# yflyzhang/RankPO

Hardware: AMD Instinct MI355X
Metric: query-passage pairs/sec (higher is better)
Workload: dtype bf16

## Files before the change

include/rankpo_hip.h:

```cpp
#ifndef RANKPO_HIP_H
#define RANKPO_HIP_H

#include <stddef.h>
#include <stdint.h>

#ifdef __cplusplus
extern "C" {
#endif

typedef void* rpo_stream_t;

typedef enum {
    RPO_OK = 0,
    RPO_ERR_INVALID_ARG = -1,
    RPO_ERR_UNSUPPORTED = -2,
    RPO_ERR_WORKSPACE = -3,
    RPO_ERR_LAUNCH = -4
} rpo_status;

typedef enum { RPO_DT_F32 = 0, RPO_DT_BF16 = 1, RPO_DT_F16 = 2 } rpo_dtype;
typedef enum { RPO_POOL_LAST = 0, RPO_POOL_CLS = 1 } rpo_pool_mode;
typedef enum { RPO_TARGET_INBATCH = 0, RPO_TARGET_FIRST = 1 } rpo_target_mode;
typedef enum { RPO_LOSS_SIGMOID = 0, RPO_LOSS_HINGE = 1 } rpo_loss_type;

// ... 70 lines not shown

typedef enum {
    RPO_LS_SCALE = 0,
    RPO_LS_MULT = 1,
    RPO_LS_NORM = 2,
    RPO_LS_SKIP = 3,
    RPO_LS_GOOD_STEPS = 4,
    RPO_LS_CUR_HYSTERESIS = 5,
    RPO_LS_APPLIED_STEPS = 6,
    RPO_LS_SKIPPED_STEPS = 7,
    RPO_LS_FLOOR_HITS = 8,
    RPO_LS_WORDS = 16
} rpo_ls_word;
int rpo_loss_scale_update(const float* sumsq, void* ls_state, float pre_scale, float max_grad_norm, int dynamic, int window,
                          int hysteresis, int consecutive_hysteresis, float min_scale, rpo_stream_t stream);
int rpo_adamw_step_scaled(void* param, float* master, const void* grad, float* exp_avg, float* exp_avg_sq, int64_t n,
                          int dtype, float lr, float beta1, float beta2, float eps, float weight_decay, const void* ls_state,
                          rpo_stream_t stream);

int rpo_swiglu_fwd(const void* g, const void* u, void* out, int64_t rows, int64_t cols, int64_t ld_gu, int64_t ld_out,
                   int dtype, rpo_stream_t stream);
int rpo_swiglu_bwd(const void* g, const void* u, const void* dout, void* dg, void* du, void* prod_out, int64_t rows,
                   int64_t cols, int64_t ld_gu, int64_t ld_dout, int64_t ld_dgu, int64_t ld_prod, int dtype,
                   rpo_stream_t stream);
int rpo_swiglu_bwd_t(const void* g, const void* u, const void* dout, void* dg, void* du, void* prod_t_out, void* dgu_t_out,
                     int64_t rows, int64_t cols, int64_t ld_gu, int64_t ld_dout, int64_t ld_dgu, int64_t ld_t, int dtype,
                     rpo_stream_t stream);
int rpo_rope(const void* x_in, void* x_out, int64_t row_stride, const float* cos_tab, const float* sin_tab,
             int64_t rows, int64_t heads, int64_t head_dim, int64_t period, int dtype, int backward,
             rpo_stream_t stream);

int rpo_transpose(const void* in, void* out, int64_t rows, int64_t cols, int64_t ld_in, int64_t ld_out, int dtype,
                  rpo_stream_t stream);

int rpo_add_rmsnorm_waves(int64_t rows);
int rpo_add_rmsnorm_fwd(const void* x, const void* delta, const void* weight, float eps, void* x_out, void* y_out,
                        float* rstd_out, int64_t rows, int64_t d, int dtype, rpo_stream_t stream);
int rpo_add_rmsnorm_bwd(const void* dy, const void* x_new, const void* weight, const float* rstd, const void* dres,
                        void* dx_out, float* dw_partial, int64_t rows, int64_t d, int dtype, rpo_stream_t stream);

int rpo_flash_attn_fwd(const void* q, const void* k, const void* v, int64_t q_stride, int64_t k_stride,
                       int64_t v_stride, const int* cu_seqlens, const int* tiles, int64_t ntiles, int64_t tile_cols,
                       int64_t total_tokens,
                       int64_t num_heads, int64_t num_kv_heads, int64_t head_dim, float scale, void* out,
                       int64_t out_stride, float* lse, int64_t lse_max_len, const float* rope_cos, const float* rope_sin,
                       int64_t rope_period, int64_t q_block, rpo_stream_t stream);

int rpo_flash_attn_bwd(const void* q, const void* k, const void* v, const void* out, const void* dout, int64_t q_stride,
                       int64_t k_stride, int64_t v_stride, int64_t out_stride, int64_t dout_stride,
                       const int* cu_seqlens, const int* q_tiles, int64_t n_q_tiles, int64_t q_tile_cols, const int* k_tiles,
                       int64_t n_k_tiles, int64_t key_block, int64_t sweep_down, int64_t total_tokens, int64_t num_heads,
                       int64_t num_kv_heads, int64_t head_dim, float scale, const float* lse, float* delta, void* dq, void* dk, void* dv,
                       int64_t dq_stride, int64_t dk_stride, int64_t dv_stride, const float* rope_cos, const float* rope_sin,
                       int64_t rope_period, int64_t q_block, rpo_stream_t stream);

int rpo_lastq_attn_fwd(const void* q, int64_t q_stride, const void* k, const void* v, int64_t k_stride, int64_t v_stride,
                       const int* cu_seqlens, int64_t num_seqs, int64_t num_heads, int64_t num_kv_heads, int64_t head_dim,
                       float scale, void* out, int64_t out_stride, float* lse, rpo_stream_t stream);
int rpo_lastq_attn_bwd(const void* q, int64_t q_stride, const void* k, const void* v, int64_t k_stride, int64_t v_stride,
                       const int* cu_seqlens, int64_t num_seqs, int64_t num_heads, int64_t num_kv_heads, int64_t head_dim,
                       float scale, const void* out, int64_t out_stride, const void* dout, int64_t dout_stride, const float* lse,
                       void* dq, int64_t dq_stride, void* dk, void* dv, int64_t dk_stride, int64_t dv_stride, rpo_stream_t stream);

int rpo_bidir_attn_fwd(const void* q, const void* k, const void* v, int64_t q_stride, int64_t k_stride, int64_t v_stride,
                       const int* cu_seqlens_q, const int* cu_seqlens_k, const int* tiles, int64_t ntiles, int64_t tile_cols,
                       int64_t q_block, int64_t total_q, int64_t num_heads, int64_t num_kv_heads, int64_t head_dim, int dtype,
// ... 94 lines not shown
```

rankpo_amd/_lib.py:

```python
from __future__ import annotations

import ctypes as C
import os

_HERE = os.path.dirname(os.path.abspath(__file__))
LIB_PATH = os.path.join(_HERE, "csrc", "librankpo_hip.so")

RPO_OK = 0
RPO_DT_F32, RPO_DT_BF16, RPO_DT_F16 = 0, 1, 2
RPO_POOL_LAST, RPO_POOL_CLS = 0, 1
(RPO_LS_SCALE, RPO_LS_MULT, RPO_LS_NORM, RPO_LS_SKIP, RPO_LS_GOOD_STEPS, RPO_LS_CUR_HYSTERESIS, RPO_LS_APPLIED_STEPS,
 RPO_LS_SKIPPED_STEPS, RPO_LS_FLOOR_HITS) = range(9)
RPO_LS_WORDS = 16
RPO_TARGET_INBATCH, RPO_TARGET_FIRST = 0, 1
RPO_LOSS_SIGMOID, RPO_LOSS_HINGE = 0, 1
RPO_BUILD_ONEWAVE64 = 1
RPO_NUM_METRICS = 9
METRIC_KEYS = (
    "rankpo_loss", "sft_loss", "rewards/chosen", "rewards/rejected", "rewards/accuracies",
    "rewards/margins", "scores/chosen", "scores/rejected", "scores/margins",
)


class RankPOParams(C.Structure):
# ... 14 lines not shown
    "rpo_version": (C.c_int, []),
    "rpo_build_flags": (C.c_int, []),
    "rpo_status_string": (C.c_char_p, [C.c_int]),
    "rpo_last_hip_error": (C.c_char_p, []),
    "rpo_pool_normalize_fwd": (C.c_int, [_vp, _i64, _i64, _vp, _i64, _i64, _i64, _i32, _i32, _i32, _f32, _vp, _vp, _vp, _vp]),
    "rpo_pool_normalize_bwd": (C.c_int, [_vp, _vp, _vp, _vp, _i64, _i64, _i64, _i32, _i32, _f32, _vp, _vp, _vp]),
    "rpo_infonce_workspace_bytes": (_sz, [_i64, _i64, _i64, _i32]),
    "rpo_infonce_debug_poison_tickets": (C.c_int, [C.c_uint64, _vp]),
    "rpo_infonce_fwd": (C.c_int, [_vp, _vp, _i64, _i64, _i64, _i32, _f32, _i32, _vp, _vp, _vp, _vp, _sz, _vp]),
    "rpo_infonce_bwd": (C.c_int, [_vp, _vp, _vp, _vp, _vp, _i64, _i64, _i64, _i32, _f32, _i32, _i64, _i64, _i64, _i64,
                                  _vp, _vp, _vp, _sz, _vp]),
    "rpo_infonce_ds": (C.c_int, [_vp, _vp, _vp, _i64, _i64, _i32, _f32, _i64, _i64, _i64, _i64, _vp, _vp, _vp]),
    "rpo_sim_gemm_nt": (C.c_int, [_vp, _i64, _i64, _vp, _i64, _i64, _i64, _vp, _i64, _vp]),
    "rpo_rankpo_fwd": (C.c_int, [_vp, _vp, _vp, _vp, _i64, _i64, _i32, C.POINTER(RankPOParams), _vp, _vp, _vp, _vp, _vp, _vp]),
    "rpo_rankpo_bwd": (C.c_int, [_vp, _vp, _vp, _vp, _i64, _i64, _i32, _vp, _vp, _vp]),
    "rpo_adamw_step": (C.c_int, [_vp, _vp, _vp, _vp, _vp, _i64, _i32, _f32, _f32, _f32, _f32, _f32, _f32, _f32, _vp, _vp]),
    "rpo_sumsq_partial": (C.c_int, [_vp, _i64, _i32, _vp, _i32, _vp]),
    "rpo_loss_scale_update": (C.c_int, [_vp, _vp, _f32, _f32, _i32, _i32, _i32, _i32, _f32, _vp]),
    "rpo_adamw_step_scaled": (C.c_int, [_vp, _vp, _vp, _vp, _vp, _i64, _i32, _f32, _f32, _f32, _f32, _f32, _vp, _vp]),
    "rpo_swiglu_fwd": (C.c_int, [_vp, _vp, _vp, _i64, _i64, _i64, _i64, _i32, _vp]),
    "rpo_topk_merge": (C.c_int, [_vp, _i64, _i64, _i64, _i64, _i32, _i32, _vp, _vp, _i32, _vp]),
    "rpo_topk_merge_split": (C.c_int, [_vp, _i64, _i64, _i64, _i64, _i32, _i32, _i32, _vp, _vp, _i32, _vp]),
    "rpo_sim_topk_filter_ok": (C.c_int, [_i64, _i64, _i64]),
    "rpo_sim_topk_filter": (C.c_int, [_vp, _vp, _i64, _i64, _i64, _i32, _i64, _i32, _i32, _vp, _vp, _vp, _vp, _vp, _i32, _vp]),
    "rpo_sim_scores_f32": (C.c_int, [_vp, _vp, _i64, _i64, _i64, _i32, _vp, _i64, _vp]),
    "rpo_topk_merge_candidates": (C.c_int, [_vp, _vp, _vp, _i64, _i32, _i32, _vp, _vp, _vp, _vp]),
    "rpo_split_bf16x3": (C.c_int, [_vp, _i64, _i64, _i64, _vp, _i64, _vp, _vp]),
    "rpo_sim_planes_ok": (C.c_int, [_i64, _i64, _i64]),
    "rpo_sim_scores_f32_planes": (C.c_int, [_vp, _vp, _i64, _i64, _i64, _vp, _i64, _vp]),
    "rpo_sim_topk_filter_planes": (C.c_int, [_vp, _vp, _i64, _i64, _i64, _i64, _i32, _vp, _vp, _vp, _vp, _vp, _i32, _vp]),
    "rpo_swiglu_bwd": (C.c_int, [_vp, _vp, _vp, _vp, _vp, _vp, _i64, _i64, _i64, _i64, _i64, _i64, _i32, _vp]),
    "rpo_swiglu_bwd_t": (C.c_int, [_vp, _vp, _vp, _vp, _vp, _vp, _vp, _i64, _i64, _i64, _i64, _i64, _i64, _i32, _vp]),
    "rpo_transpose": (C.c_int, [_vp, _vp, _i64, _i64, _i64, _i64, _i32, _vp]),
    "rpo_add_rmsnorm_waves": (C.c_int, [_i64]),
    "rpo_add_rmsnorm_fwd": (C.c_int, [_vp, _vp, _vp, _f32, _vp, _vp, _vp, _i64, _i64, _i32, _vp]),
    "rpo_add_rmsnorm_bwd": (C.c_int, [_vp, _vp, _vp, _vp, _vp, _vp, _vp, _i64, _i64, _i32, _vp]),
    "rpo_flash_attn_fwd": (C.c_int, [_vp, _vp, _vp, _i64, _i64, _i64, _vp, _vp, _i64, _i64, _i64, _i64, _i64, _i64, _f32, _vp,
                                     _i64, _vp, _i64, _vp, _vp, _i64, _i64, _vp]),
    "rpo_flash_attn_bwd": (C.c_int, [_vp] * 5 + [_i64] * 5 + [_vp, _vp, _i64, _i64, _vp, _i64, _i64, _i64, _i64, _i64, _i64, _i64, _f32, _vp, _vp,
                                     _vp, _vp, _vp, _i64, _i64, _i64, _vp, _vp, _i64, _i64, _vp]),
    "rpo_lastq_attn_fwd": (C.c_int, [_vp, _i64, _vp, _vp, _i64, _i64, _vp, _i64, _i64, _i64, _i64, _f32, _vp, _i64, _vp, _vp]),
    "rpo_lastq_attn_bwd": (C.c_int, [_vp, _i64, _vp, _vp, _i64, _i64, _vp, _i64, _i64, _i64, _i64, _f32, _vp, _i64, _vp, _i64, _vp,
                                     _vp, _i64, _vp, _vp, _i64, _i64, _vp]),
    "rpo_rope": (C.c_int, [_vp, _vp, _i64, _vp, _vp, _i64, _i64, _i64, _i64, _i32, _i32, _vp]),
    "rpo_bidir_attn_fwd": (C.c_int, [_vp, _vp, _vp, _i64, _i64, _i64, _vp, _vp, _vp, _i64, _i64, _i64, _i64, _i64, _i64, _i64, _i32,
                                     _f32, _vp, _i64, _vp, _vp]),
    "rpo_add_layernorm_fwd": (C.c_int, [_vp, _i64, _vp, _i64, _vp, _vp, _f32, _vp, _i64, _i64, _i64, _i32, _vp]),
    "rpo_gelu_fwd": (C.c_int, [_vp, _i64, _i64, _i64, _i32, _vp]),
    "rpo_bert_embed_ln_fwd": (C.c_int, [_vp, _vp, _vp, _i64, _vp, _i64, _vp, _i64, _vp, _i64, _vp, _vp, _f32, _vp, _i64, _i64, _i32,
                                        _vp]),
    "rpo_bidir_attn_fwd_f32": (C.c_int, [_vp, _vp, _vp, _i64, _i64, _i64, _vp, _vp, _vp, _i64, _i64, _i64, _i64, _i64, _i64, _i64,
                                         _f32, _vp, _i64, _vp, _vp]),
    "rpo_add_layernorm_fwd_f32": (C.c_int, [_vp, _i64, _vp, _i64, _vp, _vp, _f32, _vp, _i64, _i64, _i64, _vp]),
    "rpo_gelu_fwd_f32": (C.c_int, [_vp, _i64, _i64, _i64, _vp]),
    "rpo_bert_embed_ln_fwd_f32": (C.c_int, [_vp, _vp, _vp, _i64, _vp, _i64, _vp, _i64, _vp, _i64, _vp, _vp, _f32, _vp, _i64, _i64,
                                            _vp]),
    "rpo_bidir_attn_train_fwd": (C.c_int, [_vp, _vp, _vp, _i64, _i64, _i64, _vp, _vp, _vp, _i64, _i64, _i64, _i64, _i64, _i64, _i64,
                                           _i32, _f32, _f32, _u64, _vp, _i64, _vp, _vp]),
    "rpo_bidir_attn_bwd": (C.c_int, [_vp, _vp, _vp, _i64, _i64, _i64, _vp, _i64, _vp, _i64, _vp, _vp, _vp, _vp, _i64, _vp, _i64,
                                     _i64, _i64, _i64, _i64, _i64, _i64, _i32, _f32, _f32, _u64, _vp, _i64, _vp, _i64, _vp, _i64,
                                     _vp]),
    "rpo_bidir_attn_dropout_mask": (C.c_int, [_i64, _i64, _i64, _i64, _i64, _i64, _f32, _u64, _vp, _vp]),
    "rpo_add_layernorm_train_fwd": (C.c_int, [_vp, _i64, _vp, _i64, _vp, _vp, _f32, _vp, _i64, _vp, _i64, _i64, _i64, _i32, _vp]),
    "rpo_bert_embed_ln_train_fwd": (C.c_int, [_vp, _vp, _vp, _i64, _vp, _i64, _vp, _i64, _vp, _i64, _vp, _vp, _f32, _vp, _i64, _vp,
                                              _i64, _i64, _i32, _vp]),
    "rpo_layernorm_bwd_blocks": (C.c_int, [_i64]),
# ... 45 lines not shown
```

rankpo_amd/csrc/encoder_ops.hip:

```cpp
#include "common.hpp"

namespace {

constexpr int kEwThreads = 256;

__device__ __forceinline__ float sigmoid_f(float x) { return 1.0f / (1.0f + __expf(-x)); }

template <typename T>
__global__ __launch_bounds__(kEwThreads) void swiglu_fwd_kernel(const T* __restrict__ g, const T* __restrict__ u,
                                                                T* __restrict__ out, int64_t rows, int vec_per_row,
                                                                int64_t ld_gu, int64_t ld_out) {
    constexpr int V = Elem<T>::kVec;
    const int64_t i = (int64_t)blockIdx.x * kEwThreads + threadIdx.x;
    const int64_t r = i / vec_per_row;
    if (r >= rows) return;
    const int c = (int)(i - r * vec_per_row) * V;
    Vec16<T> a, b, o;
    a.load_nt(g + r * ld_gu + c);
    b.load_nt(u + r * ld_gu + c);
#pragma unroll
    for (int k = 0; k < V; ++k) o.v[k] = a.v[k] * sigmoid_f(a.v[k]) * b.v[k];
    o.store_nt(out + r * ld_out + c);
}

// ... 128 lines not shown
            __attribute__((aligned(16))) T v[V];
#pragma unroll
            for (int e = 0; e < V; ++e) v[e] = tile[rv + e][oc];
            if (r + V <= rows) {
                __builtin_nontemporal_store(*reinterpret_cast<const uint4_t*>(v), reinterpret_cast<uint4_t*>(out + c * ld_pt + r));
            } else {
#pragma unroll
                for (int e = 0; e < V; ++e)
                    if (r + e < rows) out[c * ld_pt + r + e] = v[e];
            }
        }
    };
    flush(prod_t);
    if constexpr (DGU_T) {
        auto refill = [&](const uint4_t* pk) {
            __syncthreads();
#pragma unroll
            for (int i = 0; i < NI; ++i) {
                const int idx = t + 256 * i;
                st_tile(&tile[idx / VPR][(idx % VPR) * V], pk[i]);
            }
        };
        refill(pk_g);
        flush(dgu_t);
        refill(pk_u);
        flush(dgu_t + cols * ld_pt);
    }
}

inline unsigned ew_grid(int64_t nvec) { return (unsigned)rpo_cdiv(nvec, kEwThreads); }

}

template <typename T>
__global__ __launch_bounds__(256) void transpose_kernel(const T* __restrict__ in, T* __restrict__ out, int64_t R, int64_t C,
                                                        int64_t ld_in, int64_t ld_out, int vec_in, int vec_out) {
    constexpr int V = 16 / (int)sizeof(T);
    constexpr int TS = 64;
    constexpr int LDT = TS + 8 / (int)sizeof(T);
    constexpr int VPR = TS / V;
    __shared__ __attribute__((aligned(16))) T tile[TS][LDT];
    const int64_t r0 = (int64_t)blockIdx.y * TS, c0 = (int64_t)blockIdx.x * TS;
    const int t = threadIdx.x;
#pragma unroll
    for (int i = 0; i < TS * VPR / 256; ++i) {
        const int idx = t + 256 * i;
        const int row = idx / VPR, cv = (idx % VPR) * V;
        const int64_t r = r0 + row, c = c0 + cv;
        __attribute__((aligned(16))) T v[V];
        if (r < R && vec_in && c + V <= C) {
            *reinterpret_cast<uint4_t*>(v) = __builtin_nontemporal_load(reinterpret_cast<const uint4_t*>(in + r * ld_in + c));
        } else {
#pragma unroll
            for (int e = 0; e < V; ++e) v[e] = (r < R && c + e < C) ? in[r * ld_in + c + e] : T(0);
        }
#pragma unroll
        for (int e = 0; e < V; ++e) tile[row][cv + e] = v[e];
    }
    __syncthreads();
#pragma unroll
    for (int i = 0; i < TS * VPR / 256; ++i) {
        const int idx = t + 256 * i;
        const int oc = idx / VPR, rv = (idx % VPR) * V;
        const int64_t c = c0 + oc, r = r0 + rv;
        if (c >= C) continue;
        __attribute__((aligned(16))) T v[V];
#pragma unroll
        for (int e = 0; e < V; ++e) v[e] = tile[rv + e][oc];
        if (vec_out && r + V <= R) {
            __builtin_nontemporal_store(*reinterpret_cast<const uint4_t*>(v), reinterpret_cast<uint4_t*>(out + c * ld_out + r));
        } else {
#pragma unroll
            for (int e = 0; e < V; ++e)
                if (r + e < R) out[c * ld_out + r + e] = v[e];
        }
    }
}

extern "C" int rpo_transpose(const void* in, void* out, int64_t rows, int64_t cols, int64_t ld_in, int64_t ld_out, int dtype,
                             rpo_stream_t stream) {
    if (!in || !out || rows <= 0 || cols <= 0 || ld_in < cols || ld_out < rows) return RPO_ERR_INVALID_ARG;
    if (!rpo_dtype_ok(dtype)) return RPO_ERR_INVALID_ARG;
    if (dtype == RPO_DT_F16) dtype = RPO_DT_BF16;
    const int64_t gx = rpo_cdiv(cols, 64), gy = rpo_cdiv(rows, 64);
    if (gy > 65535) return RPO_ERR_UNSUPPORTED;
    const int es = dtype == RPO_DT_BF16 ? 2 : 4, V = 16 / es;
    const int vec_in = rpo_aligned16(in) && (ld_in % V == 0), vec_out = rpo_aligned16(out) && (ld_out % V == 0);
    hipStream_t st = (hipStream_t)stream;
    const dim3 grid((unsigned)gx, (unsigned)gy);
    if (dtype == RPO_DT_BF16)
        RPO_LAUNCH(transpose_kernel<bf16_t>, grid, dim3(256), 0, st, (const bf16_t*)in, (bf16_t*)out, rows, cols, ld_in, ld_out,
                   vec_in, vec_out);
    else
        RPO_LAUNCH(transpose_kernel<float>, grid, dim3(256), 0, st, (const float*)in, (float*)out, rows, cols, ld_in, ld_out,
                   vec_in, vec_out);
    return rpo_launch_status();
}

extern "C" int rpo_swiglu_fwd(const void* g, const void* u, void* out, int64_t rows, int64_t cols, int64_t ld_gu,
                              int64_t ld_out, int dtype, rpo_stream_t stream) {
    if (!g || !u || !out || rows <= 0 || cols <= 0) return RPO_ERR_INVALID_ARG;
    const int V = dtype == RPO_DT_BF16 ? 8 : 4;
    if (cols % V != 0 || ld_gu % V != 0 || ld_out % V != 0 || ld_gu < cols || ld_out < cols || !rpo_aligned16(g) ||
        !rpo_aligned16(u) || !rpo_aligned16(out))
        return RPO_ERR_UNSUPPORTED;
    const int64_t nvec = rows * (cols / V);
    if (nvec / kEwThreads >= INT32_MAX) return RPO_ERR_UNSUPPORTED;
    hipStream_t st = (hipStream_t)stream;
    if (dtype == RPO_DT_BF16)
        RPO_LAUNCH(swiglu_fwd_kernel<bf16_t>, dim3(ew_grid(nvec)), dim3(kEwThreads), 0, st, (const bf16_t*)g,
                   (const bf16_t*)u, (bf16_t*)out, rows, (int)(cols / V), ld_gu, ld_out);
    else if (dtype == RPO_DT_F32)
        RPO_LAUNCH(swiglu_fwd_kernel<float>, dim3(ew_grid(nvec)), dim3(kEwThreads), 0, st, (const float*)g,
                   (const float*)u, (float*)out, rows, (int)(cols / V), ld_gu, ld_out);
    else
        return RPO_ERR_INVALID_ARG;
    return rpo_launch_status();
}

extern "C" int rpo_swiglu_bwd(const void* g, const void* u, const void* dout, void* dg, void* du, void* prod_out,
                              int64_t rows, int64_t cols, int64_t ld_gu, int64_t ld_dout, int64_t ld_dgu, int64_t ld_prod,
                              int dtype, rpo_stream_t stream) {
    if (!g || !u || !dout || !dg || !du || rows <= 0 || cols <= 0) return RPO_ERR_INVALID_ARG;
    const int V = dtype == RPO_DT_BF16 ? 8 : 4;
    if (cols % V != 0 || ld_gu % V != 0 || ld_dout % V != 0 || ld_dgu % V != 0 || !rpo_aligned16(g) ||
        !rpo_aligned16(u) || !rpo_aligned16(dout) || !rpo_aligned16(dg) || !rpo_aligned16(du) ||
        (prod_out && (ld_prod % V != 0 || !rpo_aligned16(prod_out))))
        return RPO_ERR_UNSUPPORTED;
    const int64_t nvec = rows * (cols / V);
// ... 52 lines not shown
        return RPO_ERR_UNSUPPORTED;
    const int64_t pairs = heads * ((head_dim / 2) / V);
    const int64_t rpb = pairs <= kEwThreads / 2 ? kEwThreads / pairs : 1;
    const int64_t nblk = rpo_cdiv(rows, rpb);
    int64_t grid = nblk < INT32_MAX ? nblk : INT32_MAX;
    hipStream_t st = (hipStream_t)stream;
    const float sign = backward ? -1.0f : 1.0f;
    if (dtype == RPO_DT_BF16)
        RPO_LAUNCH(rope_kernel<bf16_t>, dim3((unsigned)grid), dim3(kEwThreads), 0, st, (const bf16_t*)x_in, (bf16_t*)x, row_stride, cos_tab,
                   sin_tab, rows, (int)heads, (int)head_dim, period, sign);
    else if (dtype == RPO_DT_F32)
        RPO_LAUNCH(rope_kernel<float>, dim3((unsigned)grid), dim3(kEwThreads), 0, st, (const float*)x_in, (float*)x, row_stride, cos_tab,
                   sin_tab, rows, (int)heads, (int)head_dim, period, sign);
    else
        return RPO_ERR_INVALID_ARG;
    return rpo_launch_status();
}

namespace {

constexpr int kNormThreads = 256, kNormWaves = kNormThreads / 64;

template <typename T> struct Raw16 {
    uint4_t r;
    __device__ __forceinline__ void load_nt(const T* p) { r = __builtin_nontemporal_load(reinterpret_cast<const uint4_t*>(p)); }
    __device__ __forceinline__ void load(const T* p) { r = *reinterpret_cast<const uint4_t*>(p); }
    __device__ __forceinline__ float get(int e) const;
};
template <> __device__ __forceinline__ float Raw16<float>::get(int e) const { return __uint_as_float(r[e]); }
template <> __device__ __forceinline__ float Raw16<bf16_t>::get(int e) const {
    return (e & 1) ? __uint_as_float(r[e >> 1] & 0xffff0000u) : __uint_as_float(r[e >> 1] << 16);
}

template <typename T, int KMAX>
__global__ __launch_bounds__(kNormThreads) void add_rmsnorm_fwd_kernel(const T* __restrict__ x, const T* __restrict__ delta,
                                                                       const T* __restrict__ w, float eps,
                                                                       T* __restrict__ x_out, T* __restrict__ y,
                                                                       float* __restrict__ rstd_out, int64_t rows,
                                                                       int d, int64_t rows_per_wave) {
    constexpr int V = Elem<T>::kVec;
    const int lane = threadIdx.x & 63;
    const int64_t wave = (int64_t)blockIdx.x * kNormWaves + (threadIdx.x >> 6);
    const int nvec = d / V;
    float wv[KMAX][V];
#pragma unroll
    for (int k = 0; k < KMAX; ++k) {
        const int vi = lane + 64 * k;
        if (vi < nvec) {
            Vec16<T> t;
            t.load(w + vi * V);
#pragma unroll
            for (int e = 0; e < V; ++e) wv[k][e] = t.v[e];
        }
    }
    const int64_t r0 = wave * rows_per_wave, r1 = r0 + rows_per_wave < rows ? r0 + rows_per_wave : rows;
    const float inv_d = 1.0f / (float)d;
    for (int64_t r = r0; r < r1; ++r) {
        Vec16<T> xv[KMAX];
        float ss = 0.f;
#pragma unroll
        for (int k = 0; k < KMAX; ++k) {
            const int vi = lane + 64 * k;
            if (vi < nvec) {
                xv[k].load_nt(x + r * d + vi * V);
                if (delta) {
                    Vec16<T> dv;
                    dv.load_nt(delta + r * d + vi * V);
#pragma unroll
                    for (int e = 0; e < V; ++e) xv[k].v[e] = Elem<T>::round(xv[k].v[e] + dv.v[e]);
                    xv[k].store(x_out + r * d + vi * V);
                }
#pragma unroll
                for (int e = 0; e < V; ++e) ss = fmaf(xv[k].v[e], xv[k].v[e], ss);
            }
        }
        ss = wave_sum(ss);
        const float rstd = rsqrtf(ss * inv_d + eps);
        if (lane == 0) rstd_out[r] = rstd;
#pragma unroll
        for (int k = 0; k < KMAX; ++k) {
            const int vi = lane + 64 * k;
            if (vi < nvec) {
                Vec16<T> o;
#pragma unroll
                for (int e = 0; e < V; ++e) o.v[e] = xv[k].v[e] * rstd * wv[k][e];
                o.store(y + r * d + vi * V);
            }
        }
    }
}

template <typename T, int KMAX>
__global__ __launch_bounds__(kNormThreads) void add_rmsnorm_bwd_kernel(const T* __restrict__ dy, const T* __restrict__ xn,
                                                                       const T* __restrict__ w,
                                                                       const float* __restrict__ rstd_in,
                                                                       const T* __restrict__ dres, T* __restrict__ dx,
                                                                       float* __restrict__ dw_partial, int64_t rows,
                                                                       int d, int64_t rows_per_wave) {
    constexpr int V = Elem<T>::kVec;
    const int lane = threadIdx.x & 63;
    const int64_t wave = (int64_t)blockIdx.x * kNormWaves + (threadIdx.x >> 6);
    const int nvec = d / V;
    float dwa[KMAX][V];
    Raw16<T> wv[KMAX];
#pragma unroll
    for (int k = 0; k < KMAX; ++k) {
        const int vi = lane + 64 * k;
#pragma unroll
        for (int e = 0; e < V; ++e) dwa[k][e] = 0.f;
        if (vi < nvec) wv[k].load(w + vi * V);
    }
    const int64_t r0 = wave * rows_per_wave, r1 = r0 + rows_per_wave < rows ? r0 + rows_per_wave : rows;
    const float inv_d = 1.0f / (float)d;
    for (int64_t r = r0; r < r1; ++r) {
        const float rstd = rstd_in[r];
        Raw16<T> gv[KMAX], xv[KMAX], rv[KMAX];
        float c = 0.f;
#pragma unroll
// ... 27 lines not shown
            if (vi < nvec) {
                Vec16<T> o;
#pragma unroll
                for (int e = 0; e < V; ++e) {
                    const float xh = xv[k].get(e) * rstd;
                    const float g = gv[k].get(e) * wv[k].get(e);
                    o.v[e] = (g - xh * c) * rstd;
                }
                if (dres) {
#pragma unroll
                    for (int e = 0; e < V; ++e) o.v[e] += rv[k].get(e);
                }
                o.store(dx + r * d + vi * V);
            }
        }
    }
    if (r0 < rows || true) {
#pragma unroll
        for (int k = 0; k < KMAX; ++k) {
            const int vi = lane + 64 * k;
            if (vi < nvec) {
                Vec16<float> o;
#pragma unroll
                for (int h = 0; h < V / 4; ++h) {
#pragma unroll
                    for (int e = 0; e < 4; ++e) o.v[e] = dwa[k][4 * h + e];
                    o.store(dw_partial + wave * d + vi * V + 4 * h);
                }
            }
        }
    }
}

template <typename T>
int launch_norm_fwd(const void* x, const void* delta, const void* w, float eps, void* x_out, void* y, float* rstd,
                    int64_t rows, int64_t d, int nwaves, hipStream_t st) {
    constexpr int V = Elem<T>::kVec;
    const int kk = (int)rpo_cdiv(d / V, 64);
    const int64_t rpw = rpo_cdiv(rows, nwaves);
    const dim3 grid((unsigned)rpo_cdiv(nwaves, kNormWaves)), block(kNormThreads);
#define RPO_NF(K)                                                                                               \
    RPO_LAUNCH((add_rmsnorm_fwd_kernel<T, K>), grid, block, 0, st, (const T*)x, (const T*)delta, (const T*)w, eps, \
               (T*)x_out, (T*)y, rstd, rows, (int)d, rpw)
    if (kk <= 1) RPO_NF(1);
    else if (kk <= 2) RPO_NF(2);
    else if (kk <= 4) RPO_NF(4);
    else if (kk <= 8) RPO_NF(8);
    else if (kk <= 16) RPO_NF(16);
    else return RPO_ERR_UNSUPPORTED;
#undef RPO_NF
    return rpo_launch_status();
}

template <typename T>
int launch_norm_bwd(const void* dy, const void* xn, const void* w, const float* rstd, const void* dres, void* dx,
                    float* dwp, int64_t rows, int64_t d, int nwaves, hipStream_t st) {
    constexpr int V = Elem<T>::kVec;
    const int kk = (int)rpo_cdiv(d / V, 64);
    const int64_t rpw = rpo_cdiv(rows, nwaves);
    const dim3 grid((unsigned)rpo_cdiv(nwaves, kNormWaves)), block(kNormThreads);
#define RPO_NB(K)                                                                                                \
    RPO_LAUNCH((add_rmsnorm_bwd_kernel<T, K>), grid, block, 0, st, (const T*)dy, (const T*)xn, (const T*)w, rstd,  \
               (const T*)dres, (T*)dx, dwp, rows, (int)d, rpw)
    if (kk <= 1) RPO_NB(1);
    else if (kk <= 2) RPO_NB(2);
    else if (kk <= 4) RPO_NB(4);
    else if (kk <= 8) RPO_NB(8);
    else return RPO_ERR_UNSUPPORTED;
#undef RPO_NB
    return rpo_launch_status();
}

}

#ifndef RPO_NORM_FWD_CAP
#define RPO_NORM_FWD_CAP 8192
#endif
#ifndef RPO_NORM_BWD_CAP
#define RPO_NORM_BWD_CAP 8192
#endif
static int norm_waves(int64_t rows, int64_t cap) {
    int64_t w = rows < cap ? rows : cap;
    w = (w + 3) / 4 * 4;
    return (int)(w < 4 ? 4 : w);
}

extern "C" int rpo_add_rmsnorm_waves(int64_t rows) {
    return norm_waves(rows, RPO_NORM_BWD_CAP);
}

extern "C" int rpo_add_rmsnorm_fwd(const void* x, const void* delta, const void* weight, float eps, void* x_out,
                                   void* y_out, float* rstd_out, int64_t rows, int64_t d, int dtype,
                                   rpo_stream_t stream) {
    if (!x || !weight || !y_out || !rstd_out || rows <= 0 || d <= 0) return RPO_ERR_INVALID_ARG;
    if (delta && !x_out) return RPO_ERR_INVALID_ARG;
    const int V = dtype == RPO_DT_BF16 ? 8 : 4;
    if (d % V != 0 || !rpo_aligned16(x) || !rpo_aligned16(y_out) || !rpo_aligned16(weight) ||
        (delta && (!rpo_aligned16(delta) || !rpo_aligned16(x_out))))
        return RPO_ERR_UNSUPPORTED;
    hipStream_t st = (hipStream_t)stream;
    const int nw = norm_waves(rows, RPO_NORM_FWD_CAP);
    if (dtype == RPO_DT_BF16) return launch_norm_fwd<bf16_t>(x, delta, weight, eps, x_out, y_out, rstd_out, rows, d, nw, st);
    if (dtype == RPO_DT_F32) return launch_norm_fwd<float>(x, delta, weight, eps, x_out, y_out, rstd_out, rows, d, nw, st);
    return RPO_ERR_INVALID_ARG;
}

extern "C" int rpo_add_rmsnorm_bwd(const void* dy, const void* x_new, const void* weight, const float* rstd,
                                   const void* dres, void* dx_out, float* dw_partial, int64_t rows, int64_t d,
                                   int dtype, rpo_stream_t stream) {
    if (!dy || !x_new || !weight || !rstd || !dx_out || !dw_partial || rows <= 0 || d <= 0) return RPO_ERR_INVALID_ARG;
    const int V = dtype == RPO_DT_BF16 ? 8 : 4;
    if (d % V != 0 || !rpo_aligned16(dy) || !rpo_aligned16(x_new) || !rpo_aligned16(dx_out) || !rpo_aligned16(weight) ||
        !rpo_aligned16(dw_partial) || (dres && !rpo_aligned16(dres)))
        return RPO_ERR_UNSUPPORTED;
    hipStream_t st = (hipStream_t)stream;
    const int nw = rpo_add_rmsnorm_waves(rows);
    if (dtype == RPO_DT_BF16) return launch_norm_bwd<bf16_t>(dy, x_new, weight, rstd, dres, dx_out, dw_partial, rows, d, nw, st);
    if (dtype == RPO_DT_F32) return launch_norm_bwd<float>(dy, x_new, weight, rstd, dres, dx_out, dw_partial, rows, d, nw, st);
    return RPO_ERR_INVALID_ARG;
}
```

rankpo_amd/ops.py:

```python
from __future__ import annotations

import ctypes as C
import threading
from dataclasses import dataclass

import torch

from . import _lib
from ._lib import (RPO_DT_BF16, RPO_DT_F16, RPO_DT_F32, RPO_LOSS_HINGE, RPO_LOSS_SIGMOID, RPO_NUM_METRICS, RPO_POOL_CLS,
                   RPO_POOL_LAST, RPO_TARGET_FIRST, RPO_TARGET_INBATCH, METRIC_KEYS, RankPOParams, check)

F_NORMALIZE_EPS = 1e-12


def _dt(t: torch.Tensor) -> int:
    if t.dtype == torch.float32:
        return RPO_DT_F32
    if t.dtype == torch.bfloat16:
        return RPO_DT_BF16
    if t.dtype == torch.float16:
        return RPO_DT_F16
    raise TypeError(f"rankpo_amd HIP kernels take float32, bfloat16 or float16 tensors, got {t.dtype}")


# ... 242 lines not shown
def rankpo_loss_metrics(q, p, cfg: RankPOConfig, ref_chosen=None, ref_rejected=None):
    return _RankPO.apply(q, p, ref_chosen, ref_rejected, cfg)


def _swiglu_fwd(lib, gu, prod, rows, ff):
    es = gu.element_size()
    with torch.cuda.device(gu.device):
        check(lib.rpo_swiglu_fwd(gu.data_ptr(), gu.data_ptr() + ff * es, prod.data_ptr(), rows, ff, 2 * ff, ff, _dt(gu),
                                 _stream(gu)), "rpo_swiglu_fwd")
    return prod


LINEAR_TN = True
WGRAD_MIXED = True
SWIGLU_DGU_T = True
SWIGLU_DGU_T_DEFAULT_MAX_BYTES = 6 * 2 ** 30
SWIGLU_DGU_T_MAX_BYTES = SWIGLU_DGU_T_DEFAULT_MAX_BYTES
SWIGLU_PROD_T = True
WGRAD_SPLIT_T = 4


def transpose2d(x):
    _need_gpu(x)
    lib = _lib.load()
    if x.dim() != 2 or x.stride(1) != 1:
        raise ValueError("transpose2d: a 2-D tensor with contiguous rows")
    R, C_ = x.shape
    out = torch.empty((C_, R), dtype=x.dtype, device=x.device)
    with torch.cuda.device(x.device):
        check(lib.rpo_transpose(x.data_ptr(), out.data_ptr(), R, C_, x.stride(0), R, _dt(x), _stream(x)), "rpo_transpose")
    return out


WGRAD_DY_T_HITS = 0


def wgrad(dy2, x2, dy_t=None):
    n, k = dy2.shape[1], x2.shape[1]
    if dy_t is not None and tuple(dy_t.shape) == (n, dy2.shape[0]) and dy_t.dtype == dy2.dtype and x2.stride(1) == 1:
        global WGRAD_DY_T_HITS
        WGRAD_DY_T_HITS += 1
        return torch.nn.functional.linear(dy_t, transpose2d(x2))
    if WGRAD_MIXED and dy2.is_cuda and dy2.dtype == torch.bfloat16 and dy2.stride(1) == 1 and x2.stride(1) == 1:
        if n >= 2 * k:
            return dy2.t() @ transpose2d(x2).t()
        if k >= 2 * n:
            return transpose2d(dy2) @ x2
        T, S = dy2.shape[0], WGRAD_SPLIT_T
        if S > 1 and T >= 32768 and T % S == 0 and n * k <= 8 * 1024 * 1024 and dy2.is_contiguous() and x2.is_contiguous():
            if _bmm_f32_out_ok(dy2.device):
                part = torch.bmm(dy2.view(S, T // S, n).transpose(1, 2), x2.view(S, T // S, k), out_dtype=torch.float32)
                return part.sum(0).to(dy2.dtype)
    return dy2.t() @ x2


_BMM_F32_OUT = {}


def _bmm_f32_out_ok(device) -> bool:
    key = str(device)
    if key not in _BMM_F32_OUT:
        try:
            a = torch.ones(2, 8, 16, dtype=torch.bfloat16, device=device)
            r = torch.bmm(a.transpose(1, 2), a, out_dtype=torch.float32)
            _BMM_F32_OUT[key] = bool(r.dtype == torch.float32 and float(r[0, 0, 0]) == 8.0)
        except Exception:
            _BMM_F32_OUT[key] = False
    return _BMM_F32_OUT[key]


def _wt(w):
    return transpose2d(w) if w.is_cuda and w.dtype in (torch.bfloat16, torch.float16, torch.float32) and w.stride(1) == 1 else w.t().contiguous()


class _LinearTN(torch.autograd.Function):

    @staticmethod
    def forward(ctx, x, w):
        ctx.save_for_backward(x, w)
        return torch.nn.functional.linear(x, w)

    @staticmethod
    def backward(ctx, dy):
        x, w = ctx.saved_tensors
        dx = dw = None
# ... 1100 lines not shown
    if not search_planes_takes(qp, cp):
        raise ValueError("similarity_f32_planes: bf16 [rows, 3 d] planes of a shape the plane-walking frame takes (search_planes_takes)")
    scores = torch.empty((qp.shape[0], cp.shape[0]), dtype=torch.float32, device=qp.device)
    with torch.cuda.device(qp.device):
        check(lib.rpo_sim_scores_f32_planes(qp.data_ptr(), cp.data_ptr(), qp.shape[0], cp.shape[0], qp.shape[1] // 3, scores.data_ptr(),
                                            scores.stride(0), _stream(qp)), "rpo_sim_scores_f32_planes")
    return scores


def search_step_planes(qp, cp, col0: int, best_val, best_idx, ws: SearchWorkspace):
    _need_gpu(qp, cp)
    lib = _lib.load()
    if not search_planes_takes(qp, cp):
        raise ValueError("search_step_planes: bf16 [rows, 3 d] planes of a shape the plane-walking frame takes (search_planes_takes)")
    rows, d = qp.shape[0], qp.shape[1] // 3
    k = best_val.shape[1]
    if (ws.rows, ws.k) != (rows, k) or best_val.shape != (rows, k) or best_idx.shape != (rows, k) or not best_val.is_contiguous() \
            or not best_idx.is_contiguous() or best_val.dtype != torch.float32 or best_idx.dtype != torch.int64:
        raise ValueError("search_step_planes: best_val / best_idx must be contiguous f32 / int64 [rows, k] matching the workspace")
    with torch.cuda.device(qp.device):
        st = _stream(qp)
        check(lib.rpo_sim_topk_filter_planes(qp.data_ptr(), cp.data_ptr(), rows, cp.shape[0], d, int(col0), k, best_val.data_ptr(),
                                             best_idx.data_ptr(), ws.cand_val.data_ptr(), ws.cand_idx.data_ptr(), ws.cand_cnt.data_ptr(),
                                             ws.cap, st), "rpo_sim_topk_filter_planes")
        check(lib.rpo_topk_merge_candidates(ws.cand_val.data_ptr(), ws.cand_idx.data_ptr(), ws.cand_cnt.data_ptr(), rows, ws.cap, k,
                                            best_val.data_ptr(), best_idx.data_ptr(), ws.overflow.data_ptr(), st),
              "rpo_topk_merge_candidates")
    return best_val, best_idx


__all__ = ["sim_gemm_nt", "pool_normalize", "topk_merge", "topk_finish", "search_step", "similarity_f32", "search_filter_takes", "search_filter_ok", "SearchWorkspace",
           "split_bf16x3", "split_bf16x3_ref", "similarity_f32_planes", "search_step_planes", "search_planes_takes",
           "search_candidate_cap", "linear", "transpose2d", "wgrad", "infonce_loss", "similarity", "rankpo_loss_metrics", "RankPOConfig", "METRIC_KEYS",
           "swiglu_down", "rope_", "fused_encoder_ops_ok", "add_rmsnorm", "fused_norm_ok",
           "flash_attn_varlen", "flash_attn_varlen_qkv", "last_query_attn", "last_query_attn_ok", "rope_flash_attn_varlen_qkv", "rope_flash_attn_varlen_qkv_fwd", "flash_attn_varlen_fwd", "flash_attn_varlen_bwd", "attn_tile_table", "attn_fwd_tile_table", "recomputing",
           "attn_key_tile_table"]
```

Baseline: 55.64.

## Widen transpose tiles, pipeline add-rmsnorm rows, add fused split-K partial sum kernel

Three separate changes. The transpose kernel is templated on tile shape, and large matrices use wide tiles of 512 bytes per row so fewer, larger blocks each move more data. The add+RMSNorm forward kernel becomes a persistent grid-stride kernel sized from occupancy: it prefetches the next row's x and delta while reducing the current row, and it is specialised for full-width and delta/no-delta cases. The split-K weight-gradient reduction now uses a native kernel that sums the f32 slices and writes bf16/f16 in one pass, replacing torch sum followed by a cast and the extra round trip through memory.

```diff
diff --git a/include/rankpo_hip.h b/include/rankpo_hip.h
--- a/include/rankpo_hip.h
+++ b/include/rankpo_hip.h
@@ -126,6 +126,8 @@
 
 int rpo_transpose(const void* in, void* out, int64_t rows, int64_t cols, int64_t ld_in, int64_t ld_out, int dtype,
                   rpo_stream_t stream);
+
+int rpo_sum_partials(const float* part, void* out, int64_t slices, int64_t n, int64_t k, int dtype, rpo_stream_t stream);
 
 int rpo_add_rmsnorm_waves(int64_t rows);
 int rpo_add_rmsnorm_fwd(const void* x, const void* delta, const void* weight, float eps, void* x_out, void* y_out,
diff --git a/rankpo_amd/_lib.py b/rankpo_amd/_lib.py
--- a/rankpo_amd/_lib.py
+++ b/rankpo_amd/_lib.py
@@ -70,6 +70,7 @@
     "rpo_swiglu_bwd": (C.c_int, [_vp, _vp, _vp, _vp, _vp, _vp, _i64, _i64, _i64, _i64, _i64, _i64, _i32, _vp]),
     "rpo_swiglu_bwd_t": (C.c_int, [_vp, _vp, _vp, _vp, _vp, _vp, _vp, _i64, _i64, _i64, _i64, _i64, _i64, _i32, _vp]),
     "rpo_transpose": (C.c_int, [_vp, _vp, _i64, _i64, _i64, _i64, _i32, _vp]),
+    "rpo_sum_partials": (C.c_int, [_vp, _vp, _i64, _i64, _i64, _i32, _vp]),
     "rpo_add_rmsnorm_waves": (C.c_int, [_i64]),
     "rpo_add_rmsnorm_fwd": (C.c_int, [_vp, _vp, _vp, _f32, _vp, _vp, _vp, _i64, _i64, _i32, _vp]),
     "rpo_add_rmsnorm_bwd": (C.c_int, [_vp, _vp, _vp, _vp, _vp, _vp, _vp, _i64, _i64, _i32, _vp]),
diff --git a/rankpo_amd/csrc/encoder_ops.hip b/rankpo_amd/csrc/encoder_ops.hip
--- a/rankpo_amd/csrc/encoder_ops.hip
+++ b/rankpo_amd/csrc/encoder_ops.hip
@@ -184,18 +184,19 @@
 
 }
 
-template <typename T>
+template <typename T, int TR, int TC>
 __global__ __launch_bounds__(256) void transpose_kernel(const T* __restrict__ in, T* __restrict__ out, int64_t R, int64_t C,
                                                         int64_t ld_in, int64_t ld_out, int vec_in, int vec_out) {
     constexpr int V = 16 / (int)sizeof(T);
-    constexpr int TS = 64;
-    constexpr int LDT = TS + 8 / (int)sizeof(T);
-    constexpr int VPR = TS / V;
-    __shared__ __attribute__((aligned(16))) T tile[TS][LDT];
-    const int64_t r0 = (int64_t)blockIdx.y * TS, c0 = (int64_t)blockIdx.x * TS;
+    constexpr int LDT = TC + 8 / (int)sizeof(T);
+    constexpr int VPR = TC / V;
+    constexpr int VPC = TR / V;
+    static_assert((TR * VPR) % 256 == 0 && (TC * VPC) % 256 == 0, "whole vectors per thread");
+    __shared__ __attribute__((aligned(16))) T tile[TR][LDT];
+    const int64_t r0 = (int64_t)blockIdx.y * TR, c0 = (int64_t)blockIdx.x * TC;
     const int t = threadIdx.x;
 #pragma unroll
-    for (int i = 0; i < TS * VPR / 256; ++i) {
+    for (int i = 0; i < TR * VPR / 256; ++i) {
         const int idx = t + 256 * i;
         const int row = idx / VPR, cv = (idx % VPR) * V;
         const int64_t r = r0 + row, c = c0 + cv;
@@ -211,9 +212,9 @@
     }
     __syncthreads();
 #pragma unroll
-    for (int i = 0; i < TS * VPR / 256; ++i) {
+    for (int i = 0; i < TC * VPC / 256; ++i) {
         const int idx = t + 256 * i;
-        const int oc = idx / VPR, rv = (idx % VPR) * V;
+        const int oc = idx / VPC, rv = (idx % VPC) * V;
         const int64_t c = c0 + oc, r = r0 + rv;
         if (c >= C) continue;
         __attribute__((aligned(16))) T v[V];
@@ -227,6 +228,27 @@
                 if (r + e < R) out[c * ld_out + r + e] = v[e];
         }
     }
+}
+
+constexpr int64_t kTransposeWideMin = 2048;
+
+template <typename T, int TR, int TC>
+static int launch_transpose(const void* in, void* out, int64_t rows, int64_t cols, int64_t ld_in, int64_t ld_out, int vec_in,
+                            int vec_out, hipStream_t st) {
+    const int64_t gx = rpo_cdiv(cols, TC), gy = rpo_cdiv(rows, TR);
+    if (gy > 65535) return RPO_ERR_UNSUPPORTED;
+    RPO_LAUNCH((transpose_kernel<T, TR, TC>), dim3((unsigned)gx, (unsigned)gy), dim3(256), 0, st, (const T*)in, (T*)out, rows, cols,
+               ld_in, ld_out, vec_in, vec_out);
+    return rpo_launch_status();
+}
+
+template <typename T>
+static int transpose_dispatch(const void* in, void* out, int64_t rows, int64_t cols, int64_t ld_in, int64_t ld_out, int vec_in,
+                              int vec_out, hipStream_t st) {
+    constexpr int W = 512 / (int)sizeof(T);
+    if (rpo_cdiv(rows, 64) * rpo_cdiv(cols, W) >= kTransposeWideMin)
+        return launch_transpose<T, 64, W>(in, out, rows, cols, ld_in, ld_out, vec_in, vec_out, st);
+    return launch_transpose<T, 64, 64>(in, out, rows, cols, ld_in, ld_out, vec_in, vec_out, st);
 }
 
 extern "C" int rpo_transpose(const void* in, void* out, int64_t rows, int64_t cols, int64_t ld_in, int64_t ld_out, int dtype,
@@ -234,19 +256,11 @@
     if (!in || !out || rows <= 0 || cols <= 0 || ld_in < cols || ld_out < rows) return RPO_ERR_INVALID_ARG;
     if (!rpo_dtype_ok(dtype)) return RPO_ERR_INVALID_ARG;
     if (dtype == RPO_DT_F16) dtype = RPO_DT_BF16;
-    const int64_t gx = rpo_cdiv(cols, 64), gy = rpo_cdiv(rows, 64);
-    if (gy > 65535) return RPO_ERR_UNSUPPORTED;
     const int es = dtype == RPO_DT_BF16 ? 2 : 4, V = 16 / es;
     const int vec_in = rpo_aligned16(in) && (ld_in % V == 0), vec_out = rpo_aligned16(out) && (ld_out % V == 0);
     hipStream_t st = (hipStream_t)stream;
-    const dim3 grid((unsigned)gx, (unsigned)gy);
-    if (dtype == RPO_DT_BF16)
-        RPO_LAUNCH(transpose_kernel<bf16_t>, grid, dim3(256), 0, st, (const bf16_t*)in, (bf16_t*)out, rows, cols, ld_in, ld_out,
-                   vec_in, vec_out);
-    else
-        RPO_LAUNCH(transpose_kernel<float>, grid, dim3(256), 0, st, (const float*)in, (float*)out, rows, cols, ld_in, ld_out,
-                   vec_in, vec_out);
-    return rpo_launch_status();
+    if (dtype == RPO_DT_BF16) return transpose_dispatch<bf16_t>(in, out, rows, cols, ld_in, ld_out, vec_in, vec_out, st);
+    return transpose_dispatch<float>(in, out, rows, cols, ld_in, ld_out, vec_in, vec_out, st);
 }
 
 extern "C" int rpo_swiglu_fwd(const void* g, const void* u, void* out, int64_t rows, int64_t cols, int64_t ld_gu,
@@ -365,58 +379,81 @@
     return (e & 1) ? __uint_as_float(r[e >> 1] & 0xffff0000u) : __uint_as_float(r[e >> 1] << 16);
 }
 
-template <typename T, int KMAX>
-__global__ __launch_bounds__(kNormThreads) void add_rmsnorm_fwd_kernel(const T* __restrict__ x, const T* __restrict__ delta,
+template <typename T> __device__ __forceinline__ uint4_t pack16(const float* v);
+template <> __device__ __forceinline__ uint4_t pack16<float>(const float* v) {
+    return uint4_t{__float_as_uint(v[0]), __float_as_uint(v[1]), __float_as_uint(v[2]), __float_as_uint(v[3])};
+}
+template <> __device__ __forceinline__ uint4_t pack16<bf16_t>(const float* v) {
+    uint4_t t;
+#pragma unroll
+    for (int i = 0; i < 4; ++i) t[i] = (unsigned)f32_to_bf16(v[2 * i]) | ((unsigned)f32_to_bf16(v[2 * i + 1]) << 16);
+    return t;
+}
+
+template <typename T, int KMAX, bool FULL, bool DELTA>
+__global__ __launch_bounds__(kNormThreads, KMAX > 4 ? 1 : FULL ? 5 : 4) void add_rmsnorm_fwd_kernel(const T* __restrict__ x, const T* __restrict__ delta,
                                                                        const T* __restrict__ w, float eps,
                                                                        T* __restrict__ x_out, T* __restrict__ y,
                                                                        float* __restrict__ rstd_out, int64_t rows,
-                                                                       int d, int64_t rows_per_wave) {
+                                                                       int d, int64_t step) {
     constexpr int V = Elem<T>::kVec;
     const int lane = threadIdx.x & 63;
     const int64_t wave = (int64_t)blockIdx.x * kNormWaves + (threadIdx.x >> 6);
     const int nvec = d / V;
-    float wv[KMAX][V];
+    const int64_t r0 = wave, r1 = rows;
+    if (r0 >= r1) return;
+    Raw16<T> wv[KMAX], xr[KMAX], dr[KMAX];
+    auto request = [&](int64_t r) {
+#pragma unroll
+        for (int k = 0; k < KMAX; ++k) {
+            const int vi = lane + 64 * k;
+            if (FULL || vi < nvec) {
+                xr[k].load_nt(x + r * d + vi * V);
+                if constexpr (DELTA) dr[k].load_nt(delta + r * d + vi * V);
+            }
+        }
+    };
+    request(r0);
 #pragma unroll
     for (int k = 0; k < KMAX; ++k) {
         const int vi = lane + 64 * k;
-        if (vi < nvec) {
-            Vec16<T> t;
-            t.load(w + vi * V);
-#pragma unroll
-            for (int e = 0; e < V; ++e) wv[k][e] = t.v[e];
-        }
-    }
-    const int64_t r0 = wave * rows_per_wave, r1 = r0 + rows_per_wave < rows ? r0 + rows_per_wave : rows;
+        if (FULL || vi < nvec) wv[k].load(w + vi * V);
+    }
     const float inv_d = 1.0f / (float)d;
-    for (int64_t r = r0; r < r1; ++r) {
-        Vec16<T> xv[KMAX];
+    for (int64_t r = r0; r < r1; r += step) {
+        Raw16<T> xn[KMAX];
         float ss = 0.f;
 #pragma unroll
         for (int k = 0; k < KMAX; ++k) {
             const int vi = lane + 64 * k;
-            if (vi < nvec) {
-                xv[k].load_nt(x + r * d + vi * V);
-                if (delta) {
-                    Vec16<T> dv;
-                    dv.load_nt(delta + r * d + vi * V);
-#pragma unroll
-                    for (int e = 0; e < V; ++e) xv[k].v[e] = Elem<T>::round(xv[k].v[e] + dv.v[e]);
-                    xv[k].store(x_out + r * d + vi * V);
+            if (FULL || vi < nvec) {
+                if constexpr (DELTA) {
+                    float t[V];
+#pragma unroll
+                    for (int e = 0; e < V; ++e) t[e] = xr[k].get(e) + dr[k].get(e);
+                    xn[k].r = pack16<T>(t);
+                    *reinterpret_cast<uint4_t*>(x_out + r * d + vi * V) = xn[k].r;
+                } else {
+                    xn[k].r = xr[k].r;
                 }
-#pragma unroll
-                for (int e = 0; e < V; ++e) ss = fmaf(xv[k].v[e], xv[k].v[e], ss);
-            }
-        }
+                asm volatile("" : "+v"(xn[k].r));
+#pragma unroll
+                for (int e = 0; e < V; ++e) ss = fmaf(xn[k].get(e), xn[k].get(e), ss);
+            }
+        }
+        if (r + step < r1) request(r + step);
         ss = wave_sum(ss);
+#pragma unroll
+        for (int k = 0; k < KMAX; ++k) asm volatile("" : "+v"(xn[k].r), "+v"(wv[k].r));
         const float rstd = rsqrtf(ss * inv_d + eps);
         if (lane == 0) rstd_out[r] = rstd;
 #pragma unroll
         for (int k = 0; k < KMAX; ++k) {
             const int vi = lane + 64 * k;
-            if (vi < nvec) {
+            if (FULL || vi < nvec) {
                 Vec16<T> o;
 #pragma unroll
-                for (int e = 0; e < V; ++e) o.v[e] = xv[k].v[e] * rstd * wv[k][e];
+                for (int e = 0; e < V; ++e) o.v[e] = xn[k].get(e) * rstd * wv[k].get(e);
                 o.store(y + r * d + vi * V);
             }
         }
@@ -510,16 +547,46 @@
     }
 }
 
+template <typename T, int K, bool FULL, bool DELTA>
+int norm_fwd_resident_waves() {
+    static const int waves = [] {
+        int dev = 0, cus = 0, blocks = 0;
+        if (hipGetDevice(&dev) != hipSuccess || hipDeviceGetAttribute(&cus, hipDeviceAttributeMultiprocessorCount, dev) != hipSuccess ||
+            hipOccupancyMaxActiveBlocksPerMultiprocessor(&blocks, add_rmsnorm_fwd_kernel<T, K, FULL, DELTA>, kNormThreads, 0) != hipSuccess) {
+            (void)hipGetLastError();
+            return 0;
+        }
+        return cus * blocks * kNormWaves;
+    }();
+    return waves;
+}
+
+template <typename T, int K, bool FULL, bool DELTA>
+int64_t norm_fwd_rows_per_wave(int64_t rows, int cap_waves) {
+    const int resident = norm_fwd_resident_waves<T, K, FULL, DELTA>();
+    return rpo_cdiv(rows, resident > 0 ? resident : cap_waves);
+}
+
 template <typename T>
 int launch_norm_fwd(const void* x, const void* delta, const void* w, float eps, void* x_out, void* y, float* rstd,
-                    int64_t rows, int64_t d, int nwaves, hipStream_t st) {
+                    int64_t rows, int64_t d, int cap_waves, hipStream_t st) {
     constexpr int V = Elem<T>::kVec;
     const int kk = (int)rpo_cdiv(d / V, 64);
-    const int64_t rpw = rpo_cdiv(rows, nwaves);
-    const dim3 grid((unsigned)rpo_cdiv(nwaves, kNormWaves)), block(kNormThreads);
-#define RPO_NF(K)                                                                                               \
-    RPO_LAUNCH((add_rmsnorm_fwd_kernel<T, K>), grid, block, 0, st, (const T*)x, (const T*)delta, (const T*)w, eps, \
-               (T*)x_out, (T*)y, rstd, rows, (int)d, rpw)
+    const bool full = d == (int64_t)64 * V * (kk <= 1 ? 1 : kk <= 2 ? 2 : kk <= 4 ? 4 : kk <= 8 ? 8 : 16);
+#define RPO_NF2(K, F, D)                                                                                           \
+    do {                                                                                                           \
+        const int64_t rpw = norm_fwd_rows_per_wave<T, K, F, D>(rows, cap_waves);                                   \
+        const int64_t blocks = rpo_cdiv(rpo_cdiv(rows, rpw), kNormWaves);                                          \
+        RPO_LAUNCH((add_rmsnorm_fwd_kernel<T, K, F, D>), dim3((unsigned)blocks), dim3(kNormThreads), 0, st, (const T*)x,  \
+                   (const T*)delta, (const T*)w, eps, (T*)x_out, (T*)y, rstd, rows, (int)d, blocks * kNormWaves);   \
+    } while (0)
+#define RPO_NF(K)                                                                                                  \
+    do {                                                                                                           \
+        if (full && delta) RPO_NF2(K, true, true);                                                                 \
+        else if (full) RPO_NF2(K, true, false);                                                                    \
+        else if (delta) RPO_NF2(K, false, true);                                                                   \
+        else RPO_NF2(K, false, false);                                                                             \
+    } while (0)
     if (kk <= 1) RPO_NF(1);
     else if (kk <= 2) RPO_NF(2);
     else if (kk <= 4) RPO_NF(4);
@@ -527,6 +594,7 @@
     else if (kk <= 16) RPO_NF(16);
     else return RPO_ERR_UNSUPPORTED;
 #undef RPO_NF
+#undef RPO_NF2
     return rpo_launch_status();
 }
 
@@ -577,7 +645,7 @@
         (delta && (!rpo_aligned16(delta) || !rpo_aligned16(x_out))))
         return RPO_ERR_UNSUPPORTED;
     hipStream_t st = (hipStream_t)stream;
-    const int nw = norm_waves(rows, RPO_NORM_FWD_CAP);
+    const int nw = RPO_NORM_FWD_CAP;
     if (dtype == RPO_DT_BF16) return launch_norm_fwd<bf16_t>(x, delta, weight, eps, x_out, y_out, rstd_out, rows, d, nw, st);
     if (dtype == RPO_DT_F32) return launch_norm_fwd<float>(x, delta, weight, eps, x_out, y_out, rstd_out, rows, d, nw, st);
     return RPO_ERR_INVALID_ARG;
@@ -597,3 +665,55 @@
     if (dtype == RPO_DT_F32) return launch_norm_bwd<float>(dy, x_new, weight, rstd, dres, dx_out, dw_partial, rows, d, nw, st);
     return RPO_ERR_INVALID_ARG;
 }
+
+namespace {
+
+template <typename T, int S>
+__global__ __launch_bounds__(kEwThreads) void sum_partials_kernel(const float* __restrict__ part, T* __restrict__ out,
+                                                                  int64_t nvec4, int64_t slice) {
+    const int64_t i = (int64_t)blockIdx.x * kEwThreads + threadIdx.x;
+    if (i >= nvec4) return;
+    uint4_t v[S];
+#pragma unroll
+    for (int s = 0; s < S; ++s)
+        v[s] = __builtin_nontemporal_load(reinterpret_cast<const uint4_t*>(part + s * slice + 4 * i));
+    float a[4];
+#pragma unroll
+    for (int e = 0; e < 4; ++e) a[e] = __uint_as_float(v[0][e]);
+#pragma unroll
+    for (int s = 1; s < S; ++s) {
+#pragma unroll
+        for (int e = 0; e < 4; ++e) a[e] += __uint_as_float(v[s][e]);
+    }
+    __attribute__((aligned(8))) T o[4];
+#pragma unroll
+    for (int e = 0; e < 4; ++e) Elem<T>::st(&o[e], a[e]);
+    __builtin_nontemporal_store(*reinterpret_cast<const uint2_t*>(o), reinterpret_cast<uint2_t*>(out + 4 * i));
+}
+
+}
+
+extern "C" int rpo_sum_partials(const float* part, void* out, int64_t slices, int64_t n, int64_t k, int dtype,
+                                rpo_stream_t stream) {
+    if (!part || !out || slices <= 0 || n <= 0 || k <= 0) return RPO_ERR_INVALID_ARG;
+    if (dtype != RPO_DT_BF16 && dtype != RPO_DT_F16) return RPO_ERR_INVALID_ARG;
+    const int64_t total = n * k;
+    if (slices > 8 || total % 4 != 0 || !rpo_aligned16(part) || !rpo_aligned16(out)) return RPO_ERR_UNSUPPORTED;
+    const int64_t nvec4 = total / 4, blocks = rpo_cdiv(nvec4, kEwThreads);
+    if (blocks >= INT32_MAX) return RPO_ERR_UNSUPPORTED;
+    hipStream_t st = (hipStream_t)stream;
+#define RPO_SP(SV)                                                                                                      \
+    case SV:                                                                                                            \
+        if (dtype == RPO_DT_BF16)                                                                                       \
+            RPO_LAUNCH((sum_partials_kernel<bf16_t, SV>), dim3((unsigned)blocks), dim3(kEwThreads), 0, st, part, (bf16_t*)out,  \
+                       nvec4, total);                                                                                   \
+        else                                                                                                            \
+            RPO_LAUNCH((sum_partials_kernel<f16_t, SV>), dim3((unsigned)blocks), dim3(kEwThreads), 0, st, part, (f16_t*)out,    \
+                       nvec4, total);                                                                                   \
+        break
+    switch ((int)slices) {
+        RPO_SP(1); RPO_SP(2); RPO_SP(3); RPO_SP(4); RPO_SP(5); RPO_SP(6); RPO_SP(7); RPO_SP(8);
+    }
+#undef RPO_SP
+    return rpo_launch_status();
+}
diff --git a/rankpo_amd/ops.py b/rankpo_amd/ops.py
--- a/rankpo_amd/ops.py
+++ b/rankpo_amd/ops.py
@@ -298,6 +298,20 @@
     return out
 
 
+SUM_PARTIALS_NATIVE = True
+
+
+def sum_partials(part, dtype):
+    _need_gpu(part)
+    if part.dim() != 3 or part.dtype != torch.float32 or not part.is_contiguous() or dtype not in (torch.bfloat16, torch.float16):
+        raise ValueError("sum_partials: a contiguous float32 [S, n, k] tensor and a bf16 / f16 result")
+    S, n, k = part.shape
+    out = torch.empty((n, k), dtype=dtype, device=part.device)
+    with torch.cuda.device(part.device):
+        check(_lib.load().rpo_sum_partials(part.data_ptr(), out.data_ptr(), S, n, k, _dt(out), _stream(part)), "rpo_sum_partials")
+    return out
+
+
 WGRAD_DY_T_HITS = 0
 
 
@@ -316,7 +330,7 @@
         if S > 1 and T >= 32768 and T % S == 0 and n * k <= 8 * 1024 * 1024 and dy2.is_contiguous() and x2.is_contiguous():
             if _bmm_f32_out_ok(dy2.device):
                 part = torch.bmm(dy2.view(S, T // S, n).transpose(1, 2), x2.view(S, T // S, k), out_dtype=torch.float32)
-                return part.sum(0).to(dy2.dtype)
+                return sum_partials(part, dy2.dtype) if SUM_PARTIALS_NATIVE else part.sum(0).to(dy2.dtype)
     return dy2.t() @ x2
 
 
@@ -1483,6 +1497,6 @@
 __all__ = ["sim_gemm_nt", "pool_normalize", "topk_merge", "topk_finish", "search_step", "similarity_f32", "search_filter_takes", "search_filter_ok", "SearchWorkspace",
            "split_bf16x3", "split_bf16x3_ref", "similarity_f32_planes", "search_step_planes", "search_planes_takes",
            "search_candidate_cap", "linear", "transpose2d", "wgrad", "infonce_loss", "similarity", "rankpo_loss_metrics", "RankPOConfig", "METRIC_KEYS",
-           "swiglu_down", "rope_", "fused_encoder_ops_ok", "add_rmsnorm", "fused_norm_ok",
+           "swiglu_down", "rope_", "fused_encoder_ops_ok", "add_rmsnorm", "fused_norm_ok", "sum_partials",
            "flash_attn_varlen", "flash_attn_varlen_qkv", "last_query_attn", "last_query_attn_ok", "rope_flash_attn_varlen_qkv", "rope_flash_attn_varlen_qkv_fwd", "flash_attn_varlen_fwd", "flash_attn_varlen_bwd", "attn_tile_table", "attn_fwd_tile_table", "recomputing",
            "attn_key_tile_table"]
```

After: 55.73, median of 2. Within noise of the previous version (+0.2%).
